# tk1363704/CAREL-VAE

Hardware: AMD Instinct MI355X
Metric: clause-pairs/sec (training step) (higher is better)
Workload: dtype bf16

## Files before the change

carel_vae_amd/csrc/attention.hip:

```cpp
#include "attention_device.h"

namespace carel {

#ifndef CAREL_ATTN_ABLATE
#define CAREL_ATTN_ABLATE 0
#endif
constexpr int ATTN_BWD_LDS = 16384 + 16384 + 32768 + 1024;
constexpr int ATTN_BWD_LDS_REL = ATTN_BWD_LDS + 1024 + 4096;

template <bool REL, bool DROP>
__global__ __launch_bounds__(256, 2) void attn_fwd_kernel(AttnParams p) {
  __shared__ __attribute__((aligned(16))) char smem[2 * 16384 + 512 + (REL ? 1024 : 0)];
  char* kimg = smem;
  char* vimg = smem + 16384;
  float* maskadd = (float*)(smem + 32768);
  float* relb = (float*)(smem + 32768 + 512);
  const int lane = threadIdx.x & 63, wave = threadIdx.x >> 6;
  const int b = blockIdx.x / NH, h = blockIdx.x - b * NH;
  const int S = p.S;
  long row0; int len;
  sample_rows(p, b, row0, len);
  const int nkt = (len + 31) >> 5, rows = nkt << 5;
  const bf16_t* qbase = p.qkv + row0 * QKV_LD + h * HD;
  stage_att(qbase + HID, QKV_LD, rows, kimg);
  stage_att(qbase + 2 * HID, QKV_LD, rows, vimg);
  int masked_here = 0;
  for (int k = threadIdx.x; k < rows; k += 256) {
    const float ma = p.cu ? (k < len ? 0.f : MASK_NEG) : ((p.att_mask && p.att_mask[row0 + k] == 0) ? MASK_NEG : 0.f);
    maskadd[k] = ma;
    masked_here |= ma != 0.f;
  }
  if (REL) relb[threadIdx.x] = p.rel[h * 256 + threadIdx.x];
  const int q0 = wave * 32;
  const int hh = lane >> 5;
  bf16x8 qf[4];
  const bool qact = wave < nkt && (p.qlim == 0 || q0 < p.qlim);
  if (qact) {
#pragma unroll
    for (int s = 0; s < 4; ++s) qf[s] = load_frag_global(qbase + (long)(q0 + (lane & 31)) * QKV_LD + 16 * s + 8 * hh);
  }
  asm volatile("s_waitcnt vmcnt(0)" ::: "memory");
  const int any_masked = __syncthreads_or(masked_here);
  if (!qact) return;

  f32x16 x[4];
#pragma unroll
  for (int kt = 0; kt < 4; ++kt) {
#pragma unroll
    for (int r = 0; r < 16; ++r) x[kt][r] = 0.f;
    if (kt < nkt) {
#pragma unroll
      for (int s = 0; s < 4; ++s) x[kt] = mfma32(frag32_row(kimg, kt * 32, s), qf[s], x[kt]);
    }
  }
  float m = -INFINITY;
#pragma unroll
  for (int kt = 0; kt < 4; ++kt) {
    if (kt < nkt) {
      const bool tile_masked = p.cu ? (kt == nkt - 1 && (len & 31) != 0) : (any_masked != 0);
      if (tile_masked) {
#pragma unroll
        for (int r = 0; r < 16; ++r) {
          const int key = kt * 32 + acc32_row(r, lane);
          float v = fmaf(x[kt][r], SC2, maskadd[key]);
          if (REL) v = fmaf(relb[127 + key - (q0 + (lane & 31))], LOG2E, v);
          x[kt][r] = v;
          m = fmaxf(m, v);
        }
      } else {
#pragma unroll
        for (int r = 0; r < 16; ++r) {
          float v = x[kt][r] * SC2;
          if (REL) v = fmaf(relb[127 + kt * 32 + acc32_row(r, lane) - (q0 + (lane & 31))], LOG2E, v);
          x[kt][r] = v;
          m = fmaxf(m, v);
        }
      }
    }
  }
  m = fmaxf(m, __shfl_xor(m, 32, 64));
  float lsum = 0.f;
  const uint32_t ebase = (uint32_t)((((long)b * NH + h) * S + (q0 + (lane & 31))) * S) + (uint32_t)(4 * hh) + p.drop.idx_offset;
#pragma unroll
  for (int kt = 0; kt < 4; ++kt)
    if (kt < nkt) exp2_dropout_tile<DROP>(x[kt], m, lsum, ebase + (uint32_t)(kt * 32), p.drop);
  lsum += __shfl_xor(lsum, 32, 64);
  const bool qlive = q0 + (lane & 31) < len;
  if (hh == 0 && qlive) p.lse[((long)b * NH + h) * S + q0 + (lane & 31)] = (m + __builtin_amdgcn_logf(lsum)) * 0.6931471805599453f;
  const float inv = 1.0f / lsum;
  f32x16 o[2];
#pragma unroll
  for (int dt = 0; dt < 2; ++dt)
#pragma unroll
    for (int r = 0; r < 16; ++r) o[dt][r] = 0.f;
#pragma unroll
  for (int kt = 0; kt < 4; ++kt) {
    if (kt < nkt) {
#pragma unroll
      for (int s = 0; s < 2; ++s) {
        const bf16x8 pf = acc_as_operand(x[kt], s);
#pragma unroll
        for (int dt = 0; dt < 2; ++dt) o[dt] = mfma32(frag32_tr<true>(vimg, dt * 32, kt * 32 + 16 * s), pf, o[dt]);
      }
    }
  }
  bf16_t* crow = p.ctx + (row0 + q0 + (lane & 31)) * HID + h * HD;
  if (qlive) {
#pragma unroll
    for (int dt = 0; dt < 2; ++dt)
#pragma unroll
      for (int i = 0; i < 4; ++i) {
        const int d = dt * 32 + 8 * i + 4 * hh;
        uint2 v = {pack2bf(o[dt][4 * i] * inv, o[dt][4 * i + 1] * inv), pack2bf(o[dt][4 * i + 2] * inv, o[dt][4 * i + 3] * inv)};
        *(uint2*)(crow + d) = v;
      }
  }
}

__device__ __forceinline__ int swz_ds(int k) { return ((k & 3) << 3) | ((k >> 2) & 7); }
__device__ __forceinline__ int ds_off(int k, int q) { return k * 256 + ((((q >> 2) ^ swz_ds(k)) & 31) << 3) + (q & 3) * 2; }

template <bool REL, bool DROP>
__global__ __launch_bounds__(256, 2) void attn_bwd_kernel(AttnParams p) {
  extern __shared__ __attribute__((aligned(16))) char smem[];
  char* qimg = smem;
  char* doimg = smem + 16384;
  char* dsimg = smem + 32768;
  float* lse = (float*)(smem + 65536);
  float* delta = lse + 128;
  float* relb = (float*)(smem + ATTN_BWD_LDS);
  float* relg = relb + 256;
  const int lane = threadIdx.x & 63, wave = threadIdx.x >> 6;
  const int b = blockIdx.x / NH, h = blockIdx.x - b * NH;
  const int S = p.S;
  const long row0 = p.cu ? (long)p.cu[b] : (long)b * S;
  const int len = p.cu ? (p.cu[b + 1] - p.cu[b]) : S;
  const int nt = (len + 31) >> 5, rows = nt << 5;
  const int ntq = p.qlim ? min(nt, p.qlim >> 5) : nt;
  const bf16_t* qbase = p.qkv + row0 * QKV_LD + h * HD;
  const bf16_t* dobase = p.dctx + row0 * HID + h * HD;
  const bf16_t* obase = p.ctx + row0 * HID + h * HD;
  stage_att(qbase, QKV_LD, rows, qimg);
  stage_att(dobase, HID, rows, doimg);
  if (REL) {
    relb[threadIdx.x] = p.rel[h * 256 + threadIdx.x];
#pragma unroll
    for (int w = 0; w < 4; ++w) relg[w * 256 + threadIdx.x] = 0.f;
  }
  for (int k = threadIdx.x; k < rows; k += 256) lse[k] = k < len ? fmaxf(p.lse[((long)b * NH + h) * S + k], -1e30f) * LOG2E : INFINITY;
  {
    const int q = threadIdx.x >> 1, half = threadIdx.x & 1;
    float s = 0.f;
    if (q < len) {
      const uint4* a = (const uint4*)(dobase + (long)q * HID + half * 32);
      const uint4* c = (const uint4*)(obase + (long)q * HID + half * 32);
#pragma unroll
      for (int i = 0; i < 4; ++i) {
        const uint4 u = a[i], v = c[i];
        s += bf2f((bf16_t)(u.x & 0xffff)) * bf2f((bf16_t)(v.x & 0xffff)) + bf2f((bf16_t)(u.x >> 16)) * bf2f((bf16_t)(v.x >> 16));
        s += bf2f((bf16_t)(u.y & 0xffff)) * bf2f((bf16_t)(v.y & 0xffff)) + bf2f((bf16_t)(u.y >> 16)) * bf2f((bf16_t)(v.y >> 16));
        s += bf2f((bf16_t)(u.z & 0xffff)) * bf2f((bf16_t)(v.z & 0xffff)) + bf2f((bf16_t)(u.z >> 16)) * bf2f((bf16_t)(v.z >> 16));
        s += bf2f((bf16_t)(u.w & 0xffff)) * bf2f((bf16_t)(v.w & 0xffff)) + bf2f((bf16_t)(u.w >> 16)) * bf2f((bf16_t)(v.w >> 16));
      }
    }
    s += __shfl_xor(s, 1, 64);
    if (q < rows && half == 0) delta[q] = s;
  }
  const int hh = lane >> 5;
  const int kw = wave * 32;
  const bool active = wave < nt;
  bf16x8 kf[4], vf[4];
  if (active) {
#pragma unroll
    for (int s = 0; s < 4; ++s) {
      kf[s] = load_frag_global(qbase + HID + (long)(kw + (lane & 31)) * QKV_LD + 16 * s + 8 * hh);
      vf[s] = load_frag_global(qbase + 2 * HID + (long)(kw + (lane & 31)) * QKV_LD + 16 * s + 8 * hh);
    }
  }
  asm volatile("s_waitcnt vmcnt(0)" ::: "memory");
  __syncthreads();

  f32x16 dk[2], dv[2];
#pragma unroll
  for (int dt = 0; dt < 2; ++dt)
#pragma unroll
    for (int r = 0; r < 16; ++r) { dk[dt][r] = 0.f; dv[dt][r] = 0.f; }
  if (active) {
    const int key = kw + (lane & 31);
    const bool klive = key < len;
    const float madd = p.cu ? (klive ? 0.f : MASK_NEG) : ((p.att_mask && p.att_mask[row0 + key] == 0) ? MASK_NEG : 0.f);
    const float madd2 = madd * LOG2E;
    const uint32_t hbase = (uint32_t)(((long)b * NH + h) * S * S) + (uint32_t)(key & ~1) + (uint32_t)((16 * (lane & 1) + 4 * hh) * S) + p.drop.idx_offset;
    for (int qt = 0; qt < ntq; ++qt) {
      f32x16 sa, dp;
#pragma unroll
      for (int r = 0; r < 16; ++r) { sa[r] = 0.f; dp[r] = 0.f; }
#pragma unroll
      for (int s = 0; s < 4; ++s) {
        sa = mfma32(frag32_row(qimg, qt * 32, s), kf[s], sa);
        dp = mfma32(frag32_row(doimg, qt * 32, s), vf[s], dp);
      }
      uint32_t hown[8], hoth[8];
      const uint32_t odd = (uint32_t)lane & 1u;
      if constexpr (DROP && CAREL_ATTN_ABLATE != 1) {
#pragma unroll
        for (int j = 0; j < 8; ++j) {
          hown[j] = mix32(((hbase + (uint32_t)((qt * 32 + (j & 3) + 8 * (j >> 2)) * S)) >> 1) ^ p.drop.key);
          hoth[j] = (uint32_t)__builtin_amdgcn_update_dpp(0, (int)hown[j], 0xB1, 0xF, 0xF, true);
        }
      }
      f32x16 pd, dsv;
#pragma unroll
      for (int i = 0; i < 4; ++i) {
        const f32x4 l4 = *(const f32x4*)(lse + qt * 32 + 8 * i + 4 * hh);
        const f32x4 d4 = *(const f32x4*)(delta + qt * 32 + 8 * i + 4 * hh);
#pragma unroll
        for (int e = 0; e < 4; ++e) {
          const int r = 4 * i + e;
          float arg = fmaf(sa[r], SC2, madd2 - l4[e]);
          if (REL) arg = fmaf(relb[127 + key - (qt * 32 + 8 * i + 4 * hh + e)], LOG2E, arg);
          const float pr = CAREL_ATTN_ABLATE == 3 ? arg : __builtin_amdgcn_exp2f(arg);
          float dm = 1.0f;
          if constexpr (DROP && CAREL_ATTN_ABLATE != 1) dm = dropout_pick(p.drop, ((uint32_t)(r >> 3) == odd) ? hown[r & 7] : hoth[r & 7], odd);
          pd[r] = pr * dm;
          dsv[r] = pr * fmaf(dp[r], dm, -d4[e]);
        }
      }
      if (REL) {
#pragma unroll
        for (int r = 0; r < 16; ++r) {
          float* mine = relg + wave * 256 + 127 + key - (qt * 32 + acc32_row(r, lane));
          if (hh == 0) *mine += dsv[r];
          asm volatile("s_waitcnt lgkmcnt(0)" ::: "memory");
          if (hh == 1) *mine += dsv[r];
          asm volatile("s_waitcnt lgkmcnt(0)" ::: "memory");
        }
      }
#pragma unroll
      for (int i = 0; i < 4; ++i) {
        const int q = qt * 32 + 8 * i + 4 * hh;
        uint2 v = {pack2bf(dsv[4 * i], dsv[4 * i + 1]), pack2bf(dsv[4 * i + 2], dsv[4 * i + 3])};
        *(uint2*)(dsimg + ds_off(key, q)) = v;
      }
#pragma unroll
      for (int s = 0; s < 2; ++s) {
        const bf16x8 pf = acc_as_operand(pd, s), df = acc_as_operand(dsv, s);
#pragma unroll
        for (int dt = 0; dt < 2; ++dt) {
          dv[dt] = mfma32(frag32_tr<true>(doimg, dt * 32, qt * 32 + 16 * s), pf, dv[dt]);
          dk[dt] = mfma32(frag32_tr<true>(qimg, dt * 32, qt * 32 + 16 * s), df, dk[dt]);
        }
      }
    }
  }
  if (CAREL_ATTN_ABLATE == 2) return;
  __syncthreads();
  if (REL && threadIdx.x < 255) {
    const float g = ((relg[threadIdx.x] + relg[256 + threadIdx.x]) + relg[512 + threadIdx.x]) + relg[768 + threadIdx.x];
    p.drel[((long)b * NH + h) * 256 + threadIdx.x] += g;
  }
  stage_att(qbase + HID, QKV_LD, rows, doimg);
  char* slot = qimg + wave * 4096;
  bf16_t* out = p.dqkv + (row0 + kw) * QKV_LD + h * HD;
  if (active && CAREL_ATTN_ABLATE != 4) {
    store_rows_via_lds(dk, 0.125f, slot, out + HID, QKV_LD, kw, len);
    store_rows_via_lds(dv, 1.0f, slot, out + 2 * HID, QKV_LD, kw, len);
  }
  __builtin_amdgcn_sched_barrier(0);
  if (active && !p.cu && CAREL_ATTN_ABLATE != 4) asm volatile("s_waitcnt vmcnt(8)" ::: "memory");
  else asm volatile("s_waitcnt vmcnt(0)" ::: "memory");
  asm volatile("s_waitcnt lgkmcnt(0)" ::: "memory");
  __builtin_amdgcn_s_barrier();
  __builtin_amdgcn_sched_barrier(0);
  if (!active) return;
  f32x16 dq[2];
#pragma unroll
  for (int dt = 0; dt < 2; ++dt)
#pragma unroll
    for (int r = 0; r < 16; ++r) dq[dt][r] = 0.f;
  {
    const int g = lane >> 4, g1 = g & 1, h2 = g >> 1, qq = (lane & 15) >> 2, pp = lane & 3;
    for (int ks = 0; ks < (wave < ntq ? (rows >> 4) : 0); ++ks) {
      const int kr0 = 16 * ks + 8 * h2 + qq, kr1 = kr0 + 4;
      const int qcol = kw + 16 * g1 + 4 * pp;
      s16x4 a = __builtin_amdgcn_ds_read_tr16_b64_v4i16((CAREL_LDS s16x4*)(dsimg + ds_off(kr0, qcol)));
      s16x4 c = __builtin_amdgcn_ds_read_tr16_b64_v4i16((CAREL_LDS s16x4*)(dsimg + ds_off(kr1, qcol)));
      s16x8 bb = {a[0], a[1], a[2], a[3], c[0], c[1], c[2], c[3]};
      const bf16x8 bf = __builtin_bit_cast(bf16x8, bb);
#pragma unroll
      for (int dt = 0; dt < 2; ++dt) dq[dt] = mfma32(frag32_tr<false>(doimg, dt * 32, 16 * ks), bf, dq[dt]);
    }
  }
  if (CAREL_ATTN_ABLATE != 4) store_rows_via_lds(dq, 0.125f, slot, out, QKV_LD, kw, len);
}

}

using namespace carel;

static int attn_prepare(const carel_attn_args* a, AttnParams* p, const char* who, bool bwd) {
  if (!a) return set_error(CAREL_ERR_ARG, "%s: null args", who);
  if (a->heads != NH || a->head_dim != HD) return set_error(CAREL_ERR_SHAPE, "%s: heads/head_dim must be %d/%d", who, NH, HD);
  if (a->seq_len < 32 || a->seq_len > 512 || (a->seq_len & 31)) return set_error(CAREL_ERR_SHAPE, "%s: seq_len must be a multiple of 32 in [32, 512] (got %d)", who, a->seq_len);
  if (a->batch <= 0) return set_error(CAREL_ERR_SHAPE, "%s: batch must be positive", who);
  if (!a->qkv || !a->ctx || !a->lse) return set_error(CAREL_ERR_ARG, "%s: null tensor", who);
  if (bwd && (!a->dctx || !a->dqkv)) return set_error(CAREL_ERR_ARG, "%s: null gradient tensor", who);
  p->qkv = (const bf16_t*)a->qkv; p->att_mask = (const long*)a->attention_mask; p->ctx = (bf16_t*)a->ctx;
  p->lse = (float*)a->lse; p->dctx = (const bf16_t*)a->dctx; p->dqkv = (bf16_t*)a->dqkv;
  p->B = a->batch; p->S = a->seq_len; p->cu = (const int*)a->cu_seqlens;
  p->rel = (const float*)a->rel_bias_dist; p->drel = (float*)a->d_rel_bias_dist;
  if (a->q_rows < 0 || a->q_rows > 128 || (a->q_rows & 31)) return set_error(CAREL_ERR_ARG, "%s: q_rows must be 0, 32, 64 or 96", who);
  p->qlim = a->q_rows >= a->seq_len ? 0 : a->q_rows;
  if (bwd && p->rel && !p->drel) return set_error(CAREL_ERR_ARG, "%s: rel_bias_dist needs d_rel_bias_dist in the backward", who);
  p->drop = make_dropout(a->drop_seed, a->drop_site, a->drop_p, a->drop_idx_offset);
  if (p->drop.thresh != 0 && (a->drop_idx_offset & 1u))
    return set_error(CAREL_ERR_ARG, "%s: drop_idx_offset must be even with dropout on (got %u)", who, a->drop_idx_offset);
  if (p->drop.thresh != 0 && (uint64_t)a->batch * NH * (uint64_t)a->seq_len * a->seq_len + a->drop_idx_offset > 4294967296ull)
    return set_error(CAREL_ERR_SHAPE, "%s: the dropout element index ((b*12 + h)*S + q)*S + k + drop_idx_offset would wrap 32 bits "
                     "(batch %d, seq_len %d, offset %u): split the call", who, a->batch, a->seq_len, a->drop_idx_offset);
  return CAREL_OK;
}

extern "C" int carel_attention_fwd(const carel_attn_args* a, void* stream_) {
  hipStream_t stream = (hipStream_t)stream_;
  AttnParams p;
  int rc = attn_prepare(a, &p, "carel_attention_fwd", false);
  if (rc) return rc;
  if (p.S > 128) return attn_long_fwd(p, stream);
  ATTN_LAUNCH(attn_fwd_kernel, dim3(p.B * NH), 0, 0, stream, p);
  return check_launch("attn_fwd_kernel");
}

extern "C" int carel_attention_bwd(const carel_attn_args* a, void* stream_) {
  hipStream_t stream = (hipStream_t)stream_;
  AttnParams p;
  int rc = attn_prepare(a, &p, "carel_attention_bwd", true);
  if (rc) return rc;
  if (p.S > 128) return attn_long_bwd(p, a->workspace, a->workspace_bytes, stream);
  ATTN_DYNAMIC_LDS(attn_bwd_kernel, ATTN_BWD_LDS, ATTN_BWD_LDS_REL);
  ATTN_LAUNCH(attn_bwd_kernel, dim3(p.B * NH), ATTN_BWD_LDS, ATTN_BWD_LDS_REL, stream, p);
  return check_launch("attn_bwd_kernel");
}
```

carel_vae_amd/csrc/attention_device.h:

```cpp
#pragma once
#include "carel_hip_internal.h"

namespace carel {

constexpr int HD = 64;
constexpr int NH = 12;
constexpr int HID = NH * HD;
constexpr int QKV_LD = 3 * HID;
constexpr float MASK_NEG = -3.4028234663852886e38f;
constexpr float LOG2E = 1.4426950408889634f;
constexpr float SC2 = 0.125f * LOG2E;

__device__ __forceinline__ int f_att(int row) { return (((row >> 1) & 1) << 2) | ((row >> 2) & 3); }
__device__ __forceinline__ int att_off(int row, int chunk) { return row * 128 + ((chunk ^ f_att(row)) << 4); }

__device__ __forceinline__ void stage_att(const bf16_t* __restrict__ g, long ld, int rows, char* img) {
  const int lane = threadIdx.x & 63, wave = __builtin_amdgcn_readfirstlane(threadIdx.x >> 6);
  for (int q = wave; q < (rows >> 3); q += 4) {
    const int r = q * 8 + (lane >> 3);
    const int c = (lane & 7) ^ f_att(r);
    __builtin_amdgcn_global_load_lds(g + (long)r * ld + c * 8, (CAREL_LDS void*)(img + q * 1024), 16, 0, 0);
  }
}

__device__ __forceinline__ bf16x8 frag32_row(const char* img, int r0, int s) {
  const int l = threadIdx.x & 63;
  return *(const bf16x8*)(img + att_off(r0 + (l & 31), 2 * s + (l >> 5)));
}
template <bool PERM>
__device__ __forceinline__ bf16x8 frag32_tr(const char* img, int x0, int kb) {
  const int l = threadIdx.x & 63;
  const int g = l >> 4, hh = g >> 1, qq = (l & 15) >> 2, p = l & 3;
  const int chunk = ((x0 + 16 * (g & 1)) >> 3) + (p >> 1), sub = (p & 1) * 8;
  const int r0 = PERM ? (kb + 4 * hh + qq) : (kb + 8 * hh + qq);
  const int r1 = PERM ? (r0 + 8) : (r0 + 4);
  s16x4 a = __builtin_amdgcn_ds_read_tr16_b64_v4i16((CAREL_LDS s16x4*)(img + att_off(r0, chunk) + sub));
  s16x4 b = __builtin_amdgcn_ds_read_tr16_b64_v4i16((CAREL_LDS s16x4*)(img + att_off(r1, chunk) + sub));
  s16x8 r = {a[0], a[1], a[2], a[3], b[0], b[1], b[2], b[3]};
  return __builtin_bit_cast(bf16x8, r);
}

__device__ __forceinline__ bf16x8 acc_as_operand(const f32x16& x, int s) {
  const uint4 r = {pack2bf(x[8 * s], x[8 * s + 1]), pack2bf(x[8 * s + 2], x[8 * s + 3]), pack2bf(x[8 * s + 4], x[8 * s + 5]), pack2bf(x[8 * s + 6], x[8 * s + 7])};
  return __builtin_bit_cast(bf16x8, r);
}

__device__ __forceinline__ bf16x8 load_frag_global(const bf16_t* p) { return *(const bf16x8*)p; }

__device__ __forceinline__ void store_rows_via_lds(const f32x16 (&acc)[2], float scale, char* slot, bf16_t* grow0, long ld, int row_base, int nrows_live) {
  const int l = threadIdx.x & 63, r = l & 31, hh = l >> 5;
#pragma unroll
  for (int dt = 0; dt < 2; ++dt)
#pragma unroll
    for (int i = 0; i < 4; ++i) {
      const int d = dt * 32 + 8 * i + 4 * hh;
      const int chunk = (d >> 3) ^ ((r >> 1) & 7);
      const uint2 v = {pack2bf(acc[dt][4 * i] * scale, acc[dt][4 * i + 1] * scale), pack2bf(acc[dt][4 * i + 2] * scale, acc[dt][4 * i + 3] * scale)};
      *(uint2*)(slot + r * 128 + chunk * 16 + (d & 4) * 2) = v;
    }
  asm volatile("s_waitcnt lgkmcnt(0)" ::: "memory");
#pragma unroll
  for (int it = 0; it < 4; ++it) {
    const int row = it * 8 + (l >> 3), c = l & 7;
    const uint4 v = *(const uint4*)(slot + row * 128 + ((c ^ ((row >> 1) & 7)) << 4));
    if (row_base + row < nrows_live) *(uint4*)(grow0 + (long)row * ld + c * 8) = v;
  }
  asm volatile("s_waitcnt lgkmcnt(0)" ::: "memory");
}

struct AttnCommon {
  const bf16_t* qkv;
  const long* att_mask;
  bf16_t* ctx;
  float* lse;
  const bf16_t* dctx;
  bf16_t* dqkv;
  int B, S;
  Dropout drop;
  const int* cu;
  const float* rel;
  int qlim;
};
struct AttnParams : AttnCommon {
  float* drel;
};
namespace attn_long {
struct Params : AttnCommon {
  float* delta;
  float* drel_part;
  float* drel;
  int nqb, nkb;
};
}

__device__ __forceinline__ void sample_rows(const AttnCommon& p, int b, long& row0, int& len) {
  row0 = p.cu ? (long)p.cu[b] : (long)b * p.S;
  len = p.cu ? (p.cu[b + 1] - p.cu[b]) : p.S;
}

template <bool DROP>
__device__ __forceinline__ void exp2_dropout_tile(f32x16& x, float m, float& lsum, uint32_t e0, const Dropout& drop) {
#pragma unroll
  for (int r = 0; r < 16; r += 2) {
    const float p0 = __builtin_amdgcn_exp2f(x[r] - m), p1 = __builtin_amdgcn_exp2f(x[r + 1] - m);
    lsum += p0; lsum += p1;
    float d0 = 1.0f, d1 = 1.0f;
    if constexpr (DROP) {
      const uint32_t hsh = mix32(((e0 + (uint32_t)((r & 3) + 8 * (r >> 2))) >> 1) ^ drop.key);
      d0 = dropout_pick(drop, hsh, 0u); d1 = dropout_pick(drop, hsh, 1u);
    }
    x[r] = p0 * d0; x[r + 1] = p1 * d1;
  }
}
__device__ __forceinline__ void store_row_frags(const f32x16 (&acc)[2], float scale, bf16_t* row, int hh) {
#pragma unroll
  for (int dt = 0; dt < 2; ++dt)
#pragma unroll
    for (int i = 0; i < 4; ++i) {
      const int d = dt * 32 + 8 * i + 4 * hh;
      uint2 v = {pack2bf(acc[dt][4 * i] * scale, acc[dt][4 * i + 1] * scale), pack2bf(acc[dt][4 * i + 2] * scale, acc[dt][4 * i + 3] * scale)};
      *(uint2*)(row + d) = v;
    }
}

#define ATTN_LAUNCH(K, grid, LDS, LDS_REL, stream, p)                                             \
  do {                                                                                            \
    const bool drop_ = (p).drop.thresh != 0;                                                      \
    if ((p).rel) {                                                                                \
      if (drop_) hipLaunchKernelGGL((K<true, true>), grid, dim3(256), LDS_REL, stream, p);        \
      else hipLaunchKernelGGL((K<true, false>), grid, dim3(256), LDS_REL, stream, p);             \
    } else {                                                                                      \
      if (drop_) hipLaunchKernelGGL((K<false, true>), grid, dim3(256), LDS, stream, p);           \
      else hipLaunchKernelGGL((K<false, false>), grid, dim3(256), LDS, stream, p);                \
    }                                                                                             \
  } while (0)
#define ATTN_DYNAMIC_LDS(K, LDS, LDS_REL)                                                                                         \
  do {                                                                                                                            \
    static bool attr_set = false;                                                                                                 \
    if (!attr_set) {                                                                                                              \
      hipError_t e = hipFuncSetAttribute((const void*)K<false, false>, hipFuncAttributeMaxDynamicSharedMemorySize, LDS);          \
      if (e == hipSuccess) e = hipFuncSetAttribute((const void*)K<false, true>, hipFuncAttributeMaxDynamicSharedMemorySize, LDS); \
      if (e == hipSuccess) e = hipFuncSetAttribute((const void*)K<true, false>, hipFuncAttributeMaxDynamicSharedMemorySize, LDS_REL);\
      if (e == hipSuccess) e = hipFuncSetAttribute((const void*)K<true, true>, hipFuncAttributeMaxDynamicSharedMemorySize, LDS_REL);\
      if (e != hipSuccess) return set_error(CAREL_ERR_HIP, "carel_attention_bwd: hipFuncSetAttribute: %s", hipGetErrorString(e)); \
      attr_set = true;                                                                                                            \
    }                                                                                                                             \
  } while (0)

}
```

Before: 8414.

## Shrink attention backward LDS to raise occupancy and stage K in LDS

The attention backward kernel drops the separate 32KB dS buffer and instead writes dS into the Q/dO/K image region after a per-tile barrier, using a new swizzled layout. K is now staged in LDS rather than held in registers. The dO·O and LSE loads are issued before the staging so their latency overlaps. Launch bounds move to 3 blocks per CU for the non-relative variant. The aim is higher occupancy and lower register pressure, at the cost of an extra __syncthreads per query tile and more LDS reads for K fragments.

```diff
diff --git a/carel_vae_amd/csrc/attention.hip b/carel_vae_amd/csrc/attention.hip
--- a/carel_vae_amd/csrc/attention.hip
+++ b/carel_vae_amd/csrc/attention.hip
@@ -5,7 +5,7 @@
 #ifndef CAREL_ATTN_ABLATE
 #define CAREL_ATTN_ABLATE 0
 #endif
-constexpr int ATTN_BWD_LDS = 16384 + 16384 + 32768 + 1024;
+constexpr int ATTN_BWD_LDS = 16384 + 16384 + 16384 + 1024;
 constexpr int ATTN_BWD_LDS_REL = ATTN_BWD_LDS + 1024 + 4096;
 
 template <bool REL, bool DROP>
@@ -117,16 +117,17 @@
   }
 }
 
-__device__ __forceinline__ int swz_ds(int k) { return ((k & 3) << 3) | ((k >> 2) & 7); }
-__device__ __forceinline__ int ds_off(int k, int q) { return k * 256 + ((((q >> 2) ^ swz_ds(k)) & 31) << 3) + (q & 3) * 2; }
+__device__ __forceinline__ int ds_off(int k, int q) {
+  return ((k & 64) << 8) + (q >> 5) * 4096 + (k & 63) * 64 + (((((q & 31) >> 2) ^ (k >> 1)) & 7) << 3) + (q & 3) * 2;
+}
 
 template <bool REL, bool DROP>
-__global__ __launch_bounds__(256, 2) void attn_bwd_kernel(AttnParams p) {
+__global__ __launch_bounds__(256, REL ? 2 : 3) void attn_bwd_kernel(AttnParams p) {
   extern __shared__ __attribute__((aligned(16))) char smem[];
   char* qimg = smem;
   char* doimg = smem + 16384;
-  char* dsimg = smem + 32768;
-  float* lse = (float*)(smem + 65536);
+  char* kimg = smem + 32768;
+  float* lse = (float*)(smem + 49152);
   float* delta = lse + 128;
   float* relb = (float*)(smem + ATTN_BWD_LDS);
   float* relg = relb + 256;
@@ -140,23 +141,40 @@
   const bf16_t* qbase = p.qkv + row0 * QKV_LD + h * HD;
   const bf16_t* dobase = p.dctx + row0 * HID + h * HD;
   const bf16_t* obase = p.ctx + row0 * HID + h * HD;
+  const int kw = wave * 32;
+  const bool active = wave < nt;
+  const int dq_ = threadIdx.x >> 1, dhalf = threadIdx.x & 1;
+  uint4 da[4], dc[4];
+  if (dq_ < len) {
+    const uint4* a = (const uint4*)(dobase + (long)dq_ * HID + dhalf * 32);
+    const uint4* c = (const uint4*)(obase + (long)dq_ * HID + dhalf * 32);
+#pragma unroll
+    for (int i = 0; i < 4; ++i) { da[i] = a[i]; dc[i] = c[i]; }
+  }
+  const float lse_in = p.lse[((long)b * NH + h) * S + min((int)threadIdx.x, S - 1)];
+  float rel_in = 0.f;
+  if (REL) rel_in = p.rel[h * 256 + threadIdx.x];
+  bf16x8 vf[4];
+  if (active) {
+#pragma unroll
+    for (int s = 0; s < 4; ++s) vf[s] = load_frag_global(qbase + 2 * HID + (long)(kw + (lane & 31)) * QKV_LD + 16 * s + 8 * (lane >> 5));
+  }
   stage_att(qbase, QKV_LD, rows, qimg);
   stage_att(dobase, HID, rows, doimg);
+  stage_att(qbase + HID, QKV_LD, rows, kimg);
+  asm volatile("s_waitcnt vmcnt(0)" ::: "memory");
   if (REL) {
-    relb[threadIdx.x] = p.rel[h * 256 + threadIdx.x];
+    relb[threadIdx.x] = rel_in;
 #pragma unroll
     for (int w = 0; w < 4; ++w) relg[w * 256 + threadIdx.x] = 0.f;
   }
-  for (int k = threadIdx.x; k < rows; k += 256) lse[k] = k < len ? fmaxf(p.lse[((long)b * NH + h) * S + k], -1e30f) * LOG2E : INFINITY;
+  if ((int)threadIdx.x < rows) lse[threadIdx.x] = (int)threadIdx.x < len ? fmaxf(lse_in, -1e30f) * LOG2E : INFINITY;
   {
-    const int q = threadIdx.x >> 1, half = threadIdx.x & 1;
     float s = 0.f;
-    if (q < len) {
-      const uint4* a = (const uint4*)(dobase + (long)q * HID + half * 32);
-      const uint4* c = (const uint4*)(obase + (long)q * HID + half * 32);
+    if (dq_ < len) {
 #pragma unroll
       for (int i = 0; i < 4; ++i) {
-        const uint4 u = a[i], v = c[i];
+        const uint4 u = da[i], v = dc[i];
         s += bf2f((bf16_t)(u.x & 0xffff)) * bf2f((bf16_t)(v.x & 0xffff)) + bf2f((bf16_t)(u.x >> 16)) * bf2f((bf16_t)(v.x >> 16));
         s += bf2f((bf16_t)(u.y & 0xffff)) * bf2f((bf16_t)(v.y & 0xffff)) + bf2f((bf16_t)(u.y >> 16)) * bf2f((bf16_t)(v.y >> 16));
         s += bf2f((bf16_t)(u.z & 0xffff)) * bf2f((bf16_t)(v.z & 0xffff)) + bf2f((bf16_t)(u.z >> 16)) * bf2f((bf16_t)(v.z >> 16));
@@ -164,18 +182,7 @@
       }
     }
     s += __shfl_xor(s, 1, 64);
-    if (q < rows && half == 0) delta[q] = s;
-  }
-  const int hh = lane >> 5;
-  const int kw = wave * 32;
-  const bool active = wave < nt;
-  bf16x8 kf[4], vf[4];
-  if (active) {
-#pragma unroll
-    for (int s = 0; s < 4; ++s) {
-      kf[s] = load_frag_global(qbase + HID + (long)(kw + (lane & 31)) * QKV_LD + 16 * s + 8 * hh);
-      vf[s] = load_frag_global(qbase + 2 * HID + (long)(kw + (lane & 31)) * QKV_LD + 16 * s + 8 * hh);
-    }
+    if (dq_ < rows && dhalf == 0) delta[dq_] = s;
   }
   asm volatile("s_waitcnt vmcnt(0)" ::: "memory");
   __syncthreads();
@@ -185,70 +192,87 @@
   for (int dt = 0; dt < 2; ++dt)
 #pragma unroll
     for (int r = 0; r < 16; ++r) { dk[dt][r] = 0.f; dv[dt][r] = 0.f; }
+  float madd2 = 0.f;
   if (active) {
     const int key = kw + (lane & 31);
     const bool klive = key < len;
     const float madd = p.cu ? (klive ? 0.f : MASK_NEG) : ((p.att_mask && p.att_mask[row0 + key] == 0) ? MASK_NEG : 0.f);
-    const float madd2 = madd * LOG2E;
-    const uint32_t hbase = (uint32_t)(((long)b * NH + h) * S * S) + (uint32_t)(key & ~1) + (uint32_t)((16 * (lane & 1) + 4 * hh) * S) + p.drop.idx_offset;
+    madd2 = madd * LOG2E;
+  }
+  {
+    const uint32_t hbase0 = (uint32_t)(((long)b * NH + h) * S * S) + p.drop.idx_offset;
     for (int qt = 0; qt < ntq; ++qt) {
-      f32x16 sa, dp;
-#pragma unroll
-      for (int r = 0; r < 16; ++r) { sa[r] = 0.f; dp[r] = 0.f; }
-#pragma unroll
-      for (int s = 0; s < 4; ++s) {
-        sa = mfma32(frag32_row(qimg, qt * 32, s), kf[s], sa);
-        dp = mfma32(frag32_row(doimg, qt * 32, s), vf[s], dp);
-      }
-      uint32_t hown[8], hoth[8];
-      const uint32_t odd = (uint32_t)lane & 1u;
-      if constexpr (DROP && CAREL_ATTN_ABLATE != 1) {
-#pragma unroll
-        for (int j = 0; j < 8; ++j) {
-          hown[j] = mix32(((hbase + (uint32_t)((qt * 32 + (j & 3) + 8 * (j >> 2)) * S)) >> 1) ^ p.drop.key);
-          hoth[j] = (uint32_t)__builtin_amdgcn_update_dpp(0, (int)hown[j], 0xB1, 0xF, 0xF, true);
-        }
-      }
-      f32x16 pd, dsv;
-#pragma unroll
-      for (int i = 0; i < 4; ++i) {
-        const f32x4 l4 = *(const f32x4*)(lse + qt * 32 + 8 * i + 4 * hh);
-        const f32x4 d4 = *(const f32x4*)(delta + qt * 32 + 8 * i + 4 * hh);
-#pragma unroll
-        for (int e = 0; e < 4; ++e) {
-          const int r = 4 * i + e;
-          float arg = fmaf(sa[r], SC2, madd2 - l4[e]);
-          if (REL) arg = fmaf(relb[127 + key - (qt * 32 + 8 * i + 4 * hh + e)], LOG2E, arg);
-          const float pr = CAREL_ATTN_ABLATE == 3 ? arg : __builtin_amdgcn_exp2f(arg);
-          float dm = 1.0f;
-          if constexpr (DROP && CAREL_ATTN_ABLATE != 1) dm = dropout_pick(p.drop, ((uint32_t)(r >> 3) == odd) ? hown[r & 7] : hoth[r & 7], odd);
-          pd[r] = pr * dm;
-          dsv[r] = pr * fmaf(dp[r], dm, -d4[e]);
-        }
-      }
-      if (REL) {
-#pragma unroll
-        for (int r = 0; r < 16; ++r) {
-          float* mine = relg + wave * 256 + 127 + key - (qt * 32 + acc32_row(r, lane));
-          if (hh == 0) *mine += dsv[r];
-          asm volatile("s_waitcnt lgkmcnt(0)" ::: "memory");
-          if (hh == 1) *mine += dsv[r];
-          asm volatile("s_waitcnt lgkmcnt(0)" ::: "memory");
-        }
-      }
-#pragma unroll
-      for (int i = 0; i < 4; ++i) {
-        const int q = qt * 32 + 8 * i + 4 * hh;
-        uint2 v = {pack2bf(dsv[4 * i], dsv[4 * i + 1]), pack2bf(dsv[4 * i + 2], dsv[4 * i + 3])};
-        *(uint2*)(dsimg + ds_off(key, q)) = v;
-      }
-#pragma unroll
-      for (int s = 0; s < 2; ++s) {
-        const bf16x8 pf = acc_as_operand(pd, s), df = acc_as_operand(dsv, s);
-#pragma unroll
-        for (int dt = 0; dt < 2; ++dt) {
-          dv[dt] = mfma32(frag32_tr<true>(doimg, dt * 32, qt * 32 + 16 * s), pf, dv[dt]);
-          dk[dt] = mfma32(frag32_tr<true>(qimg, dt * 32, qt * 32 + 16 * s), df, dk[dt]);
+      f32x16 dsv;
+      int ln = lane;
+      asm volatile("" : "+v"(ln));
+      const int hh = ln >> 5, key = kw + (ln & 31);
+      if (active) {
+        const uint32_t hbase = hbase0 + (uint32_t)(key & ~1) + (uint32_t)((qt * 32 + 16 * (ln & 1) + 4 * hh) * S);
+        f32x16 sa, dp;
+#pragma unroll
+        for (int r = 0; r < 16; ++r) { sa[r] = 0.f; dp[r] = 0.f; }
+#pragma unroll
+        for (int s = 0; s < 4; ++s) {
+          sa = mfma32(frag32_row(qimg, qt * 32, s, ln), frag32_row(kimg, kw, s, ln), sa);
+          dp = mfma32(frag32_row(doimg, qt * 32, s, ln), vf[s], dp);
+        }
+        const uint32_t odd = (uint32_t)ln & 1u;
+        f32x16 pd;
+#pragma unroll
+        for (int u = 0; u < 2; ++u) {
+          uint32_t hown[4], hoth[4];
+          if constexpr (DROP && CAREL_ATTN_ABLATE != 1) {
+#pragma unroll
+            for (int e = 0; e < 4; ++e) {
+              hown[e] = mix32(((hbase + (uint32_t)((e + 8 * u) * S)) >> 1) ^ p.drop.key);
+              hoth[e] = (uint32_t)__builtin_amdgcn_update_dpp(0, (int)hown[e], 0xB1, 0xF, 0xF, true);
+            }
+          }
+#pragma unroll
+          for (int i = u; i < 4; i += 2) {
+            const f32x4 l4 = *(const f32x4*)(lse + qt * 32 + 8 * i + 4 * hh);
+            const f32x4 d4 = *(const f32x4*)(delta + qt * 32 + 8 * i + 4 * hh);
+#pragma unroll
+            for (int e = 0; e < 4; ++e) {
+              const int r = 4 * i + e;
+              float arg = fmaf(sa[r], SC2, madd2 - l4[e]);
+              if (REL) arg = fmaf(relb[127 + key - (qt * 32 + 8 * i + 4 * hh + e)], LOG2E, arg);
+              const float pr = CAREL_ATTN_ABLATE == 3 ? arg : __builtin_amdgcn_exp2f(arg);
+              float dm = 1.0f;
+              if constexpr (DROP && CAREL_ATTN_ABLATE != 1) dm = dropout_pick(p.drop, ((uint32_t)(i >> 1) == odd) ? hown[e] : hoth[e], odd);
+              pd[r] = pr * dm;
+              dsv[r] = pr * fmaf(dp[r], dm, -d4[e]);
+            }
+          }
+        }
+        if (REL) {
+#pragma unroll
+          for (int r = 0; r < 16; ++r) {
+            float* mine = relg + wave * 256 + 127 + key - (qt * 32 + acc32_row(r, ln));
+            if (hh == 0) *mine += dsv[r];
+            asm volatile("s_waitcnt lgkmcnt(0)" ::: "memory");
+            if (hh == 1) *mine += dsv[r];
+            asm volatile("s_waitcnt lgkmcnt(0)" ::: "memory");
+          }
+        }
+#pragma unroll
+        for (int s = 0; s < 2; ++s) {
+          const bf16x8 pf = acc_as_operand(pd, s), df = acc_as_operand(dsv, s);
+#pragma unroll
+          for (int dt = 0; dt < 2; ++dt) {
+            dv[dt] = mfma32(frag32_tr<true>(doimg, dt * 32, qt * 32 + 16 * s, ln), pf, dv[dt]);
+            dk[dt] = mfma32(frag32_tr<true>(qimg, dt * 32, qt * 32 + 16 * s, ln), df, dk[dt]);
+          }
+        }
+      }
+      asm volatile("s_waitcnt lgkmcnt(0)" ::: "memory");
+      __syncthreads();
+      if (active) {
+#pragma unroll
+        for (int i = 0; i < 4; ++i) {
+          const int q = qt * 32 + 8 * i + 4 * hh;
+          uint2 v = {pack2bf(dsv[4 * i], dsv[4 * i + 1]), pack2bf(dsv[4 * i + 2], dsv[4 * i + 3])};
+          *(uint2*)(smem + ds_off(key, q)) = v;
         }
       }
     }
@@ -259,19 +283,6 @@
     const float g = ((relg[threadIdx.x] + relg[256 + threadIdx.x]) + relg[512 + threadIdx.x]) + relg[768 + threadIdx.x];
     p.drel[((long)b * NH + h) * 256 + threadIdx.x] += g;
   }
-  stage_att(qbase + HID, QKV_LD, rows, doimg);
-  char* slot = qimg + wave * 4096;
-  bf16_t* out = p.dqkv + (row0 + kw) * QKV_LD + h * HD;
-  if (active && CAREL_ATTN_ABLATE != 4) {
-    store_rows_via_lds(dk, 0.125f, slot, out + HID, QKV_LD, kw, len);
-    store_rows_via_lds(dv, 1.0f, slot, out + 2 * HID, QKV_LD, kw, len);
-  }
-  __builtin_amdgcn_sched_barrier(0);
-  if (active && !p.cu && CAREL_ATTN_ABLATE != 4) asm volatile("s_waitcnt vmcnt(8)" ::: "memory");
-  else asm volatile("s_waitcnt vmcnt(0)" ::: "memory");
-  asm volatile("s_waitcnt lgkmcnt(0)" ::: "memory");
-  __builtin_amdgcn_s_barrier();
-  __builtin_amdgcn_sched_barrier(0);
   if (!active) return;
   f32x16 dq[2];
 #pragma unroll
@@ -283,15 +294,23 @@
     for (int ks = 0; ks < (wave < ntq ? (rows >> 4) : 0); ++ks) {
       const int kr0 = 16 * ks + 8 * h2 + qq, kr1 = kr0 + 4;
       const int qcol = kw + 16 * g1 + 4 * pp;
-      s16x4 a = __builtin_amdgcn_ds_read_tr16_b64_v4i16((CAREL_LDS s16x4*)(dsimg + ds_off(kr0, qcol)));
-      s16x4 c = __builtin_amdgcn_ds_read_tr16_b64_v4i16((CAREL_LDS s16x4*)(dsimg + ds_off(kr1, qcol)));
+      s16x4 a = __builtin_amdgcn_ds_read_tr16_b64_v4i16((CAREL_LDS s16x4*)(smem + ds_off(kr0, qcol)));
+      s16x4 c = __builtin_amdgcn_ds_read_tr16_b64_v4i16((CAREL_LDS s16x4*)(smem + ds_off(kr1, qcol)));
       s16x8 bb = {a[0], a[1], a[2], a[3], c[0], c[1], c[2], c[3]};
       const bf16x8 bf = __builtin_bit_cast(bf16x8, bb);
 #pragma unroll
-      for (int dt = 0; dt < 2; ++dt) dq[dt] = mfma32(frag32_tr<false>(doimg, dt * 32, 16 * ks), bf, dq[dt]);
-    }
-  }
-  if (CAREL_ATTN_ABLATE != 4) store_rows_via_lds(dq, 0.125f, slot, out, QKV_LD, kw, len);
+      for (int dt = 0; dt < 2; ++dt) dq[dt] = mfma32(frag32_tr<false>(kimg, dt * 32, 16 * ks), bf, dq[dt]);
+    }
+  }
+  asm volatile("s_waitcnt lgkmcnt(0)" ::: "memory");
+  __builtin_amdgcn_sched_barrier(0);
+  char* slot = qimg + wave * 4096;
+  bf16_t* out = p.dqkv + (row0 + kw) * QKV_LD + h * HD;
+  if (CAREL_ATTN_ABLATE != 4) {
+    store_rows_via_lds(dq, 0.125f, slot, out, QKV_LD, kw, len);
+    store_rows_via_lds(dk, 0.125f, slot, out + HID, QKV_LD, kw, len);
+    store_rows_via_lds(dv, 1.0f, slot, out + 2 * HID, QKV_LD, kw, len);
+  }
 }
 
 }
diff --git a/carel_vae_amd/csrc/attention_device.h b/carel_vae_amd/csrc/attention_device.h
--- a/carel_vae_amd/csrc/attention_device.h
+++ b/carel_vae_amd/csrc/attention_device.h
@@ -23,13 +23,12 @@
   }
 }
 
-__device__ __forceinline__ bf16x8 frag32_row(const char* img, int r0, int s) {
-  const int l = threadIdx.x & 63;
+__device__ __forceinline__ bf16x8 frag32_row(const char* img, int r0, int s, int l) {
   return *(const bf16x8*)(img + att_off(r0 + (l & 31), 2 * s + (l >> 5)));
 }
+__device__ __forceinline__ bf16x8 frag32_row(const char* img, int r0, int s) { return frag32_row(img, r0, s, threadIdx.x & 63); }
 template <bool PERM>
-__device__ __forceinline__ bf16x8 frag32_tr(const char* img, int x0, int kb) {
-  const int l = threadIdx.x & 63;
+__device__ __forceinline__ bf16x8 frag32_tr(const char* img, int x0, int kb, int l) {
   const int g = l >> 4, hh = g >> 1, qq = (l & 15) >> 2, p = l & 3;
   const int chunk = ((x0 + 16 * (g & 1)) >> 3) + (p >> 1), sub = (p & 1) * 8;
   const int r0 = PERM ? (kb + 4 * hh + qq) : (kb + 8 * hh + qq);
@@ -39,6 +38,8 @@
   s16x8 r = {a[0], a[1], a[2], a[3], b[0], b[1], b[2], b[3]};
   return __builtin_bit_cast(bf16x8, r);
 }
+template <bool PERM>
+__device__ __forceinline__ bf16x8 frag32_tr(const char* img, int x0, int kb) { return frag32_tr<PERM>(img, x0, kb, threadIdx.x & 63); }
 
 __device__ __forceinline__ bf16x8 acc_as_operand(const f32x16& x, int s) {
   const uint4 r = {pack2bf(x[8 * s], x[8 * s + 1]), pack2bf(x[8 * s + 2], x[8 * s + 3]), pack2bf(x[8 * s + 4], x[8 * s + 5]), pack2bf(x[8 * s + 6], x[8 * s + 7])};
```

Result: no change. 8474 (median of 6 runs) (+0.7%).
